# pmh47/dirt

Hardware: AMD Instinct MI355X
Metric: forward+backward Mpixels/s at 1024x1024x4ch, 10k-tri mesh (higher is better)
Workload: dtype f32 (f64 edge functions); 1 GPU; K3: rand_mesh F=10000 at 1024x1024x4, 1 scene(s) per GPU, forward+backward; scenes_per_gpu=1, parallelism=batch-sharded x1, no collective, launch=eager (Python wrapper + C ABI per step)

## Files before the change

### dirt_amd/csrc/dirt_device.h

```cpp
#pragma once
#include <hip/hip_runtime.h>
#include <stdint.h>

namespace dirt {

struct alignas(128) FaceRec {
    double coef[9];
    double inv_det;
    uint32_t flags;
    int32_t vid[3];
    double zp[3];
    uint32_t pad0;
    uint32_t pad1;
};
static_assert(sizeof(FaceRec) == 128, "FaceRec must be 128 bytes");
constexpr int FACE_SHADE_BYTES = 96;

constexpr uint32_t FACE_VALID = 0x80000000u;

struct alignas(8) FaceBox {
    int16_t i_min, i_max, r_min, r_max;
};
static_assert(sizeof(FaceBox) == 8, "FaceBox must be 8 bytes");

constexpr uint32_t Z24_CLEAR = 0x00FFFFFFu;

__device__ __forceinline__ void face_fetch_indices(const int32_t* __restrict__ face, int32_t (&idx)[3])
{
    idx[0] = face[0]; idx[1] = face[1]; idx[2] = face[2];
}
__device__ __forceinline__ void face_fetch_vertices(const float* __restrict__ verts, int V, const int32_t (&idx)[3], float4 (&vv)[3])
{
#pragma unroll
    for (int k = 0; k < 3; ++k)
        vv[k] = V > 0 ? *reinterpret_cast<const float4*>(verts + (size_t)((uint32_t)idx[k] < (uint32_t)V ? idx[k] : 0) * 4) : make_float4(0.f, 0.f, 0.f, 0.f);
}
__device__ inline bool setup_face_from(const float4 (&vv)[3], const int32_t (&idx)[3], int V, int H, int W, FaceRec& rec, FaceBox& box);

__device__ inline bool setup_face(const float* __restrict__ verts, int V, const int32_t* __restrict__ face,
                                  int H, int W, FaceRec& rec, FaceBox& box)
{
    int32_t idx[3];
    float4 vv[3];
    face_fetch_indices(face, idx);
    face_fetch_vertices(verts, V, idx, vv);
    return setup_face_from(vv, idx, V, H, W, rec, box);
}

__device__ inline bool setup_face_edges(const float4 (&vv)[3], const int32_t (&idx)[3], int V, int H, int W, FaceRec& rec)
{
    double X[3], Y[3], Wc[3], Z[3];
    const int32_t i0 = idx[0], i1 = idx[1], i2 = idx[2];
    const bool index_ok = ((uint32_t)i0 < (uint32_t)V) & ((uint32_t)i1 < (uint32_t)V) & ((uint32_t)i2 < (uint32_t)V);
    if (V <= 0) return false;
    if (!index_ok) return false;
#pragma unroll
    for (int k = 0; k < 3; ++k) {
        const int32_t vi = k == 0 ? i0 : (k == 1 ? i1 : i2);
        const float4 v = vv[k];
        if (!(isfinite(v.x) && isfinite(v.y) && isfinite(v.z) && isfinite(v.w))) return false;
        X[k] = ((double)v.x + (double)v.w) * (0.5 * (double)W);
        Y[k] = ((double)v.y + (double)v.w) * (0.5 * (double)H);
        Wc[k] = (double)v.w;
        Z[k] = (double)v.z;
        rec.vid[k] = vi;
    }
    double a[3], b[3], c[3];
#pragma unroll
    for (int k = 0; k < 3; ++k) {
        const int p = (k + 1) % 3, q = (k + 2) % 3;
        double m1, m2;
        m1 = Y[p] * Wc[q]; m2 = Wc[p] * Y[q]; a[k] = m1 - m2;
        m1 = Wc[p] * X[q]; m2 = X[p] * Wc[q]; b[k] = m1 - m2;
        m1 = X[p] * Y[q];  m2 = Y[p] * X[q];  c[k] = m1 - m2;
    }
    const double t0 = X[0] * a[0], t1 = Y[0] * b[0], t2 = Wc[0] * c[0];
    double det = (t0 + t1) + t2;
    if (!isfinite(det) || det == 0.0) return false;
    if (det < 0.0) {
#pragma unroll
        for (int k = 0; k < 3; ++k) { a[k] = -a[k]; b[k] = -b[k]; c[k] = -c[k]; }
        det = -det;
    }
    const double inv_det = 1.0 / det;
    if (!isfinite(inv_det)) return false;

    double zs[3];
#pragma unroll
    for (int k = 0; k < 3; ++k) zs[k] = Z[k] * inv_det;
    {
        double m0, m1, m2;
        m0 = a[0] * zs[0]; m1 = a[1] * zs[1]; m2 = a[2] * zs[2]; rec.zp[0] = ((m0 + m1) + m2) * 8388607.5;
        m0 = b[0] * zs[0]; m1 = b[1] * zs[1]; m2 = b[2] * zs[2]; rec.zp[1] = ((m0 + m1) + m2) * 8388607.5;
        m0 = c[0] * zs[0]; m1 = c[1] * zs[1]; m2 = c[2] * zs[2]; rec.zp[2] = fma((m0 + m1) + m2, 8388607.5, 8388607.5);
    }
    uint32_t flags = FACE_VALID;
#pragma unroll
    for (int k = 0; k < 3; ++k) {
        const bool incl = (a[k] > 0.0) || (a[k] == 0.0 && b[k] > 0.0);
        if (!incl) { a[k] = -a[k]; b[k] = -b[k]; c[k] = -c[k]; flags |= (1u << k); }
        rec.coef[3 * k + 0] = a[k]; rec.coef[3 * k + 1] = b[k]; rec.coef[3 * k + 2] = c[k];
    }
    rec.flags = flags; rec.pad0 = 0; rec.pad1 = 0;
    rec.inv_det = inv_det;
    return true;
}

__device__ inline bool setup_face_box(const float4 (&vv)[3], int H, int W, FaceBox& box)
{
    double X[3], Y[3], Wc[3], Z[3];
#pragma unroll
    for (int k = 0; k < 3; ++k) {
        const float4 v = vv[k];
        X[k] = ((double)v.x + (double)v.w) * (0.5 * (double)W);
        Y[k] = ((double)v.y + (double)v.w) * (0.5 * (double)H);
        Wc[k] = (double)v.w;
        Z[k] = (double)v.z;
    }
    const int npos = (Wc[0] > 0.0) + (Wc[1] > 0.0) + (Wc[2] > 0.0);
    if (npos == 0) return false;
    int i_min = 0, i_max = W - 1, j_min = 0, j_max = H - 1;
    if (npos == 3) {
        if (Z[0] > Wc[0] && Z[1] > Wc[1] && Z[2] > Wc[2]) return false;
        if (Z[0] < -Wc[0] && Z[1] < -Wc[1] && Z[2] < -Wc[2]) return false;
        float xmin = INFINITY, xmax = -INFINITY, ymin = INFINITY, ymax = -INFINITY;
#pragma unroll
        for (int k = 0; k < 3; ++k) {
            const float rw = 1.0f / (float)Wc[k];
            float xw = (float)X[k] * rw, yw = (float)Y[k] * rw;
            if (!(fabsf(xw) <= 32768.f)) xw = xw > 0.f ? 32768.f : -32768.f;
            if (!(fabsf(yw) <= 32768.f)) yw = yw > 0.f ? 32768.f : -32768.f;
            xmin = fminf(xmin, xw); xmax = fmaxf(xmax, xw);
            ymin = fminf(ymin, yw); ymax = fmaxf(ymax, yw);
        }
        if (!(xmin <= xmax) || !(ymin <= ymax)) { xmin = ymin = -32768.f; xmax = ymax = 32768.f; }
        const float d = 1.0f / 32.0f;
        float lo, hi;
        lo = ceilf(fmaxf(xmin - 0.5f - d, -1.0f)); hi = floorf(fminf(xmax - 0.5f + d, (float)W));
        if (lo > (float)i_min) i_min = (int)lo;
        if (hi < (float)i_max) i_max = (int)hi;
        lo = ceilf(fmaxf(ymin - 0.5f - d, -1.0f)); hi = floorf(fminf(ymax - 0.5f + d, (float)H));
        if (lo > (float)j_min) j_min = (int)lo;
        if (hi < (float)j_max) j_max = (int)hi;
    }
    if (i_min > i_max || j_min > j_max) return false;
    box.i_min = (int16_t)i_min; box.i_max = (int16_t)i_max;
    box.r_min = (int16_t)(H - 1 - j_max); box.r_max = (int16_t)(H - 1 - j_min);
    return true;
}

__device__ inline bool setup_face_from(const float4 (&vv)[3], const int32_t (&idx)[3], int V, int H, int W, FaceRec& rec, FaceBox& box)
{
    if (!setup_face_edges(vv, idx, V, H, W, rec)) return false;
    return setup_face_box(vv, H, W, box);
}

__device__ inline void edge_eval(const double* coef, double px, double py, double F[3])
{
    F[0] = fma(coef[0], px, fma(coef[1], py, coef[2]));
    F[1] = fma(coef[3], px, fma(coef[4], py, coef[5]));
    F[2] = fma(coef[6], px, fma(coef[7], py, coef[8]));
}

__device__ inline void bary_eval(const double F[3], uint32_t flags, double inv_det, float b[3], float& clip_w)
{
    const double s0 = (flags & 1u) ? -inv_det : inv_det;
    const double s1 = (flags & 2u) ? -inv_det : inv_det;
    const double s2 = (flags & 4u) ? -inv_det : inv_det;
    const float l0 = (float)(F[0] * s0), l1 = (float)(F[1] * s1), l2 = (float)(F[2] * s2);
    const float s = (l0 + l1) + l2;
    const float r = 1.0f / s;
    b[0] = l0 * r; b[1] = l1 * r; b[2] = l2 * r;
    clip_w = r;
}

__device__ __forceinline__ float2 encode_bary(float b0, float b1, float b2)
{
    const bool omit2 = (b2 >= b0) & (b2 >= b1);
    const bool omit0 = !omit2 & (b0 >= b1);
    const bool omit1 = !omit2 & !omit0;
    const float p = omit2 ? b0 : (omit0 ? b1 : b2);
    const float q = omit2 ? b1 : (omit0 ? b2 : b0);
    return make_float2(__uint_as_float(__float_as_uint(p) | (omit0 ? 0x80000000u : 0u)),
                       __uint_as_float(__float_as_uint(q) | (omit1 ? 0x80000000u : 0u)));
}
__device__ __forceinline__ void decode_bary(float2 e, float (&b)[3])
{
    const bool sp = (int32_t)__float_as_uint(e.x) < 0, sq = (int32_t)__float_as_uint(e.y) < 0;
    const float P = fabsf(e.x), Q = fabsf(e.y);
    const float d = (1.f - P) - Q;
    b[0] = sq ? Q : (sp ? d : P);
    b[1] = sq ? d : (sp ? P : Q);
    b[2] = sq ? P : (sp ? Q : d);
}

__device__ __forceinline__ int xcd_tile(int b, int ntiles)
{
    const int x = b & 7, j = b >> 3;
    const int q = ntiles >> 3, rem = ntiles & 7;
    return x * q + min(x, rem) + j;
}

inline uint32_t tile_magic(int tiles_x) { return tiles_x <= 1 ? 0u : (uint32_t)(0x100000000ull / (uint32_t)tiles_x) + 1u; }
__device__ __forceinline__ void tile_xy(int tile, int tiles_x, uint32_t magic, int& tx, int& ty)
{
    ty = magic ? (int)__umulhi((uint32_t)tile, magic) : tile;
    tx = tile - ty * tiles_x;
}

}
```

### dirt_amd/csrc/dirt_forward.hip

```cpp
#include "dirt_device.h"
#include "dirt_launch.h"
#include "dirt_raster_common.h"
#include "../../include/dirt_hip.h"

namespace dirt {

#ifdef DIRT_TRACE
__device__ long long* g_trace_fwd_setup = nullptr;
__device__ long long* g_trace_fwd_raster = nullptr;
extern "C" void dirt_debug_set_trace_forward(void* ps, void* pr)
{
    long long* q = reinterpret_cast<long long*>(ps);
    (void)hipMemcpyToSymbol(HIP_SYMBOL(g_trace_fwd_setup), &q, sizeof(q));
    q = reinterpret_cast<long long*>(pr);
    (void)hipMemcpyToSymbol(HIP_SYMBOL(g_trace_fwd_raster), &q, sizeof(q));
}
#define FMARK() do { if (tr_n < 12) { long long t_; asm volatile("s_memtime %0\n\ts_waitcnt lgkmcnt(0)" : "=s"(t_) :: "memory"); tr_t[tr_n++] = t_; } } while (0)
#define FTRACE_DECL() long long tr_t[12]; int tr_n = 0; const long long tr_wall0 = wall_clock64()
#else
#define FMARK() do {} while (0)
#define FTRACE_DECL() do {} while (0)
#endif

namespace {

constexpr int MAX_FACE_BINS = 16;

__device__ __forceinline__ void glds16(const void* base, uint32_t voff, uint32_t lds_addr)
{
    unsigned keep;
    asm volatile("s_mov_b32 %0, m0\n\ts_mov_b32 m0, %3\n\ts_nop 0\n\tglobal_load_lds_dwordx4 %1, %2\n\ts_mov_b32 m0, %0"
                 : "=&s"(keep) : "v"(voff), "s"(base), "s"(lds_addr) : "memory");
}

struct Float3v { float x, y, z; };

template <class T>
__device__ __forceinline__ uint32_t lds_address(T* p)
{
    return (uint32_t)(uintptr_t)(__attribute__((address_space(3))) void*)p;
}

}

constexpr int STHREADS = 256;
template <int CK>
__global__ __launch_bounds__(STHREADS) void setup_kernel_v2(const float* __restrict__ a_vertices, const int32_t* __restrict__ a_faces,
                                                            const float* __restrict__ a_vertex_colors, int a_shared_faces, int a_V, int a_F,
                                                            GeomParams g_in)
{
    GeomParams g = g_in;
    g.vertices = a_vertices; g.faces = a_faces; g.vertex_colors = a_vertex_colors; g.shared_faces = a_shared_faces; g.V = a_V; g.F = a_F;
    __shared__ __align__(16) unsigned long long s_mask[MAX_BINS_MASKED + 2];
    __shared__ __align__(16) FaceRec s_recs[64];
    __shared__ __align__(16) TileRec s_lrecs[64];
    __shared__ __align__(16) float4 s_crecs[CK ? 3 * 64 : 1];
    __shared__ FaceBox s_box[64];
    __shared__ uint8_t s_ok_edges[64], s_ok_box[64];
    const int ib = blockIdx.y, chunk = blockIdx.x, tid = threadIdx.x, lane = tid & 63;
    const int role = __builtin_amdgcn_readfirstlane(tid >> 6);
    FTRACE_DECL();
    FMARK();
    const int nbins = g.grid.bins_x * g.grid.bins_y, big = g.grid.big;
    BinCell* __restrict__ row = g.cells + ((size_t)ib * g.nchunk + chunk) * (size_t)g.grid.cell_chunk_stride;
    if (g.F == 0 || g.V <= 0) {
        for (int i = tid; i <= big; i += STHREADS) if (i < nbins || i == big) row[i] = BinCell{0u, 0u};
        return;
    }
    const int f0 = chunk * 64;
    const int nf = min(64, g.F - f0);
    const size_t n0 = (size_t)ib * g.F + f0;
    const int f = f0 + lane;
    const bool have = lane < nf;
    const int fs = have ? f : 0;
    const float* __restrict__ verts = g.vertices + (size_t)ib * g.V * 4;
    const float* __restrict__ cols = CK ? g.vertex_colors + (size_t)ib * g.V * CK : nullptr;
    auto fetch = [&](int vid) {
        if (role != 3) return *reinterpret_cast<const float4*>(verts + (size_t)vid * 4);
        if constexpr (CK == 0) return make_float4(0.f, 0.f, 0.f, 0.f);
        else {
            const float* __restrict__ cp = cols + (size_t)vid * CK;
            if constexpr (CK == 4) return *reinterpret_cast<const float4*>(cp);
            else if constexpr (CK == 3) { const Float3v q = *reinterpret_cast<const Float3v*>(cp); return make_float4(q.x, q.y, q.z, 0.f); }
            else return make_float4(cp[0], 0.f, 0.f, 0.f);
        }
    };
    int32_t idx[3] = {0, 0, 0};
    float4 vv[3];
    const bool fetches = role != 2 && (role != 3 || CK != 0);
    if (fetches) {
        const int32_t* __restrict__ fp = g.faces + (g.shared_faces ? (size_t)fs : (size_t)ib * g.F + fs) * 3;
        idx[0] = fp[0]; idx[1] = fp[1]; idx[2] = fp[2];
#pragma unroll
        for (int k = 0; k < 3; ++k) vv[k] = fetch(min(3 * fs + k, g.V - 1));
    } else if (role == 2) {
        for (int i = lane; i < nbins; i += 64) s_mask[i] = 0ull;
        if (lane == 0) s_mask[big] = 0ull;
    }
    FMARK();
    if (fetches) {
        const bool identity = 3 * fs + 2 < g.V && idx[0] == 3 * fs && idx[1] == 3 * fs + 1 && idx[2] == 3 * fs + 2;
        if (__builtin_amdgcn_ballot_w64(have && !identity) != 0ull) {
#pragma unroll
            for (int k = 0; k < 3; ++k) {
                const int ci = identity ? 3 * fs + k : ((uint32_t)idx[k] < (uint32_t)g.V ? idx[k] : 0);
                vv[k] = fetch(ci);
            }
        }
    }
    FMARK();
    bool ok_mine = false;
    FaceBox box;
    box.i_min = 0; box.i_max = -1; box.r_min = 0; box.r_max = -1;
    if (role == 0) {
        FaceRec rec;
        ok_mine = have && setup_face_edges(vv, idx, g.V, g.H, g.W, rec);
        if (ok_mine) s_recs[lane] = rec;
        else s_recs[lane].flags = 0;
        s_ok_edges[lane] = ok_mine ? 1 : 0;
    } else if (role == 1) {
        ok_mine = have && setup_face_box(vv, g.H, g.W, box);
        s_box[lane] = box;
        s_ok_box[lane] = ok_mine ? 1 : 0;
    } else if (role == 3) {
        if constexpr (CK != 0) { s_crecs[3 * lane] = vv[0]; s_crecs[3 * lane + 1] = vv[1]; s_crecs[3 * lane + 2] = vv[2]; }
    }
    FMARK();
    __syncthreads();
    if (role == 1) {
        if (ok_mine && s_ok_edges[lane]) {
            const unsigned long long bit = 1ull << lane;
            const int bx0 = box.i_min >> g.grid.shift, bx1 = box.i_max >> g.grid.shift;
            const int by0 = box.r_min >> g.grid.shift, by1 = box.r_max >> g.grid.shift;
            if ((bx1 - bx0 + 1) * (by1 - by0 + 1) <= MAX_FACE_BINS) {
                for (int by = by0; by <= by1; ++by)
                    for (int bx = bx0; bx <= bx1; ++bx) atomicOr(&s_mask[by * g.grid.bins_x + bx], bit);
            } else {
                atomicOr(&s_mask[big], bit);
            }
            if (!g.v2_only) {
                BinEntry e;
                e.box = box; e.face = f; e.pad = 0;
                g.entries[((size_t)ib * g.nchunk + chunk) * (5 * (size_t)g.chunk_faces) + lane] = e;
            }
        }
    } else if (role == 2) {
        if (have && s_ok_edges[lane] && s_ok_box[lane]) {
            TileRec lr;
            make_local_rec(s_recs[lane], f, s_box[lane], g.H, (float)g.W, (float)g.H, &lr);
            s_lrecs[lane] = lr;
        }
    } else if (role == 0) {
        const uint4* __restrict__ src = reinterpret_cast<const uint4*>(&s_recs[0]);
        uint4* __restrict__ dst = reinterpret_cast<uint4*>(g.recs + n0);
        for (int i = lane; i < 8 * nf; i += 64) dst[i] = src[i];
    } else {
        if constexpr (CK != 0) {
            const uint4* __restrict__ src = reinterpret_cast<const uint4*>(&s_crecs[0]);
            uint4* __restrict__ dst = reinterpret_cast<uint4*>(g.crecs + 3 * n0);
            for (int i = lane; i < 3 * nf; i += 64) dst[i] = src[i];
        }
    }
    __syncthreads();
    FMARK();
    {
        const uint4* __restrict__ src = reinterpret_cast<const uint4*>(&s_lrecs[0]);
        uint4* __restrict__ dst = reinterpret_cast<uint4*>(g.lrecs + n0);
        for (int i = tid; i < 5 * nf; i += STHREADS) dst[i] = src[i];
    }
    for (int i = 2 * tid; i < nbins; i += 2 * STHREADS) {
        if (i + 1 < nbins) {
            const ulonglong2 m = *reinterpret_cast<const ulonglong2*>(&s_mask[i]);
            *reinterpret_cast<ulonglong2*>(&row[i]) = m;
        } else {
            const unsigned long long m = s_mask[i];
            row[i] = BinCell{(uint32_t)m, (uint32_t)(m >> 32)};
        }
    }
    if (tid == STHREADS - 1) {
        const unsigned long long m = s_mask[big];
        row[big] = BinCell{(uint32_t)m, (uint32_t)(m >> 32)};
    }
    FMARK();
#ifdef DIRT_TRACE
    if (tid == 0 && g_trace_fwd_setup) {
        long long* o = g_trace_fwd_setup + ((size_t)blockIdx.y * gridDim.x + blockIdx.x) * 16;
        for (int i = 0; i < 12; ++i) o[i] = i < tr_n ? tr_t[i] : 0;
        o[12] = tr_wall0; o[13] = (long long)wall_clock64() - tr_wall0;
    }
#endif
}

hipError_t launch_geometry_v2(const GeomParams& g, hipStream_t stream)
{
    const dim3 grid((unsigned)g.nchunk, (unsigned)g.B);
    const int ck = g.crecs ? g.C : 0;
    if (ck == 4) hipLaunchKernelGGL(setup_kernel_v2<4>, grid, dim3(STHREADS), 0, stream, g.vertices, g.faces, g.vertex_colors, g.shared_faces, g.V, g.F, g);
    else if (ck == 3) hipLaunchKernelGGL(setup_kernel_v2<3>, grid, dim3(STHREADS), 0, stream, g.vertices, g.faces, g.vertex_colors, g.shared_faces, g.V, g.F, g);
    else if (ck == 1) hipLaunchKernelGGL(setup_kernel_v2<1>, grid, dim3(STHREADS), 0, stream, g.vertices, g.faces, g.vertex_colors, g.shared_faces, g.V, g.F, g);
    else hipLaunchKernelGGL(setup_kernel_v2<0>, grid, dim3(STHREADS), 0, stream, g.vertices, g.faces, g.vertex_colors, g.shared_faces, g.V, g.F, g);
    return hipGetLastError();
}

namespace {

#ifndef DIRT_V2_CAP
#define DIRT_V2_CAP 96
#endif
constexpr int V2_CAP = DIRT_V2_CAP;

template <bool COLOURS>
struct alignas(16) ShadeSlot {
    double coef[9];
    double inv_det;
    uint32_t flags;
    int32_t vid[3];
    float4 col[COLOURS ? 3 : 0];
};
static_assert(sizeof(ShadeSlot<true>) == 144 && sizeof(ShadeSlot<false>) == 96, "16-byte pieces: 6 of the record, 3 colours");

}

#ifndef DIRT_V2_WAVES
#define DIRT_V2_WAVES 6
#endif
template <int MODE, int CSPEC, int WAVES = 4>
__global__ __launch_bounds__(64 * WAVES, WAVES == 8 ? 8 : DIRT_V2_WAVES) void raster_kernel_v2(
    const BinCell* __restrict__ a_cells, int a_nchunk, int a_tiles_x, int a_tiles_y, uint32_t a_tiles_x_magic, int a_shift, int a_bins_x,
    int a_big, int a_chunk_stride, RasterParams p_in)
{
    RasterParams p = p_in;
    p.cells = a_cells; p.nchunk = a_nchunk; p.tiles_x = a_tiles_x; p.tiles_y = a_tiles_y; p.tiles_x_magic = a_tiles_x_magic;
    p.grid.shift = a_shift; p.grid.bins_x = a_bins_x; p.grid.big = a_big; p.grid.cell_chunk_stride = a_chunk_stride;
    constexpr int NB = 2, NBY = WAVES == 8 ? 1 : 2, TILE = 32, PPL = NB * NBY, THREADS = 64 * WAVES, RH = 8 * NBY;
    constexpr bool COLOURS = MODE == 0;
    constexpr int SPARTS = COLOURS ? 9 : 6;
    using Slot = ShadeSlot<COLOURS>;
    __shared__ __align__(16) TileRec s_rec[V2_CAP];
    __shared__ __align__(16) Slot s_shade[V2_CAP];
    __shared__ int32_t s_face[V2_CAP];
    __shared__ uint32_t s_count;
    FTRACE_DECL();
    FMARK();
#ifdef DIRT_TRACE
    int tr_cand = 0;
#endif
    const int tid = threadIdx.x;
    const int lane = tid & 63;
    const int wave = __builtin_amdgcn_readfirstlane(tid >> 6);
    const int ib = blockIdx.y;
    const int tile = xcd_tile(blockIdx.x, p.tiles_x * p.tiles_y);
    int tile_col, tile_row;
    tile_xy(tile, p.tiles_x, p.tiles_x_magic, tile_col, tile_row);
    const int tx0 = tile_col * TILE, tr0 = tile_row * TILE;
    constexpr int C = CSPEC;

    const FaceRec* __restrict__ recs = p.recs + (size_t)ib * p.F;
    const TileRec* __restrict__ lrecs = p.lrecs + (size_t)ib * p.F;
    const float4* __restrict__ crecs = COLOURS ? p.crecs + (size_t)ib * p.F * 3 : nullptr;
    const int bin = (tr0 >> p.grid.shift) * p.grid.bins_x + (tx0 >> p.grid.shift);
    const BinCell* __restrict__ cells = p.cells + (size_t)ib * p.nchunk * (size_t)p.grid.cell_chunk_stride;
    unsigned long long m_bin = 0ull, m_big = 0ull;
    if (tid < p.nchunk) {
        const BinCell* __restrict__ rowc = cells + (size_t)tid * p.grid.cell_chunk_stride;
        const BinCell a = rowc[bin], b = rowc[p.grid.big];
        m_bin = ((unsigned long long)a.count << 32) | a.start;
        m_big = ((unsigned long long)b.count << 32) | b.start;
    }

    const int wx = wave & 1, wy = wave >> 1;
    const int x0 = tx0 + wx * 16 + (lane & 7);
    const int r0 = tr0 + wy * RH + (lane >> 3);
    double px[NB], py[NBY];
#pragma unroll
    for (int k = 0; k < NB; ++k) px[k] = (double)(x0 + 8 * k) + 0.5;
#pragma unroll
    for (int k = 0; k < NBY; ++k) py[k] = (double)(p.H - 1 - (r0 + 8 * k)) + 0.5;
    unsigned long long best[PPL];
    int cbest[PPL];
#pragma unroll
    for (int k = 0; k < PPL; ++k) { best[k] = (unsigned long long)Z24_CLEAR << 32; cbest[k] = V2_CAP; }
    bool lds_records = true;

    if ((p.zero_b_bytes | p.zero_c_bytes) != 0) {
        const unsigned gwg = blockIdx.y * gridDim.x + blockIdx.x;
        if (p.zero_b_bytes) zero_share<THREADS>(p.zero_b, p.zero_b_bytes, p.zero_b_per, gwg, tid);
        if (p.zero_c_bytes) zero_share<THREADS>(p.zero_c, p.zero_c_bytes, p.zero_c_per, gwg, tid);
    }
    const uint32_t lds_rec = (uint32_t)__builtin_amdgcn_readfirstlane((int)lds_address(&s_rec[0]));
    const uint32_t lds_shade = (uint32_t)__builtin_amdgcn_readfirstlane((int)lds_address(&s_shade[0]));

    FMARK();
    for (int round = 0;; ++round) {
        if (tid == 0) s_count = 0;
        __syncthreads();
        FMARK();
        {
            const uint32_t cnt = (uint32_t)__popcll(m_bin) + (uint32_t)__popcll(m_big);
            uint32_t incl = cnt;
            incl += (uint32_t)__builtin_amdgcn_update_dpp(0, (int)incl, 0x111 , 0xF, 0xF, false);
            incl += (uint32_t)__builtin_amdgcn_update_dpp(0, (int)incl, 0x112 , 0xF, 0xF, false);
            incl += (uint32_t)__builtin_amdgcn_update_dpp(0, (int)incl, 0x114 , 0xF, 0xF, false);
            incl += (uint32_t)__builtin_amdgcn_update_dpp(0, (int)incl, 0x118 , 0xF, 0xF, false);
            incl += (uint32_t)__builtin_amdgcn_update_dpp(0, (int)incl, 0x142 , 0xA, 0xF, false);
            incl += (uint32_t)__builtin_amdgcn_update_dpp(0, (int)incl, 0x143 , 0xC, 0xF, false);
            const uint32_t total = (uint32_t)__builtin_amdgcn_readlane((int)incl, 63);
            uint32_t base = 0;
            if (total != 0u) {
                if (lane == 0) base = atomicAdd(&s_count, total);
                base = (uint32_t)__builtin_amdgcn_readfirstlane((int)base);
            }
            uint32_t slot = base + incl - cnt;
            const int face0 = tid * 64;
            while (m_bin != 0ull && slot < (uint32_t)V2_CAP) {
                s_face[slot++] = face0 + (__ffsll((long long)m_bin) - 1);
                m_bin &= m_bin - 1ull;
            }
            while (m_big != 0ull && slot < (uint32_t)V2_CAP) {
                s_face[slot++] = face0 + (__ffsll((long long)m_big) - 1);
                m_big &= m_big - 1ull;
            }
        }
        FMARK();
        __syncthreads();
        FMARK();
        const int n = (int)min(s_count, (uint32_t)V2_CAP);
        if (round != 0) lds_records = false;

        int tid_o = tid;
        asm volatile("" : "+v"(tid_o));
#pragma unroll
        for (int k = 0; k < (5 * V2_CAP + THREADS - 1) / THREADS; ++k) {
            const int idx = tid_o + THREADS * k;
            if (idx < 5 * n) {
                const int slot = idx / 5, part = idx - 5 * slot;
                glds16(lrecs, (uint32_t)s_face[slot] * (uint32_t)sizeof(TileRec) + 16u * (uint32_t)part, lds_rec + 1024u * (uint32_t)(wave + WAVES * k));
            }
        }
        asm volatile("s_waitcnt vmcnt(0)" ::: "memory");
        FMARK();
        __syncthreads();
        FMARK();
        if (round == 0) {
#pragma unroll
            for (int k = 0; k < (SPARTS * V2_CAP + THREADS - 1) / THREADS; ++k) {
                const int idx = tid_o + THREADS * k;
                if (idx < SPARTS * n) {
                    const int slot = idx / SPARTS, part = idx - SPARTS * slot;
                    const uint32_t face = (uint32_t)s_face[slot];
                    const uint32_t dst = lds_shade + 1024u * (uint32_t)(wave + WAVES * k);
                    if (part < 6) glds16(recs, face * (uint32_t)sizeof(FaceRec) + 16u * (uint32_t)part, dst);
                    if (COLOURS && part >= 6) glds16(crecs, face * 48u + 16u * (uint32_t)(part - 6), dst);
                }
            }
        }

        for (int cb = 0; cb < n; cb += 64) {
            const int idx = cb + lane;
            uint32_t mym4 = 0;
            if (idx < n) {
                const FaceBox box = s_rec[idx].box;
                const int rx0 = tx0 + 16 * wx, ry0 = tr0 + RH * wy;
                const int bx0 = max(box.i_min - rx0, 0) >> 3, bx1 = min(box.i_max - rx0, 15) >> 3;
                const int by0 = max(box.r_min - ry0, 0) >> 3, by1 = min(box.r_max - ry0, RH - 1) >> 3;
                if (box.i_max >= rx0 && box.i_min <= rx0 + 15 && box.r_max >= ry0 && box.r_min <= ry0 + RH - 1) {
                    const uint32_t rowbits = (bx0 == 0 ? 1u : 0u) | (bx1 == 1 ? 2u : 0u);
                    mym4 = (by0 == 0 ? rowbits : 0u) | (NBY == 2 && by1 == 1 ? rowbits << 2 : 0u);
                    mym4 = cull_blocks<NB, NBY>(s_rec[idx], mym4, (float)(rx0 - (int)box.i_min), (float)((int)box.r_min - ry0));
                }
            }
            unsigned long long m = __builtin_amdgcn_ballot_w64(mym4 != 0);
            auto visit = [&](const TileRec& t, int k) {
                const uint32_t m4 = (uint32_t)__builtin_amdgcn_readlane((int)mym4, k);
                float dxl[NB], dyl[NBY];
#pragma unroll
                for (int q = 0; q < NB; ++q) dxl[q] = (float)(x0 + 8 * q - (int)t.box.i_min);
#pragma unroll
                for (int q = 0; q < NBY; ++q) dyl[q] = (float)((int)t.box.r_min - (r0 + 8 * q));
                raster_candidate<NB, NBY>(t, recs, round == 0 ? cb + k : V2_CAP, m4, dxl, dyl, px, py, best, cbest);
#ifdef DIRT_TRACE
                ++tr_cand;
#endif
            };
            while (m) {
                const int k = __ffsll((long long)m) - 1;
                m &= m - 1;
                const TileRec t = s_rec[cb + k];
                visit(t, k);
            }
        }
        FMARK();
        asm volatile("s_waitcnt vmcnt(0)" ::: "memory");
        const bool more = (m_bin | m_big) != 0ull;
        if (!__syncthreads_or(more)) break;
    }
    FMARK();

    int32_t fbest[PPL];
#pragma unroll
    for (int k = 0; k < PPL; ++k) fbest[k] = (uint32_t)(best[k] >> 32) != Z24_CLEAR ? (int32_t)(uint32_t)best[k] : -1;

    constexpr bool BG_FIRST = WAVES != 8;
    const float* __restrict__ cols = COLOURS ? p.vertex_colors + (size_t)ib * p.V * C : nullptr;
    int xs0 = x0, rs0 = r0;
    asm volatile("" : "+v"(xs0), "+v"(rs0));
    auto pixel_index = [&](int k, bool& inside) {
        const int x = xs0 + 8 * (k % NB), r = rs0 + 8 * (k / NB);
        inside = x < p.W && r < p.H;
        return ((size_t)ib * p.H + min(r, p.H - 1)) * p.W + min(x, p.W - 1);
    };
    auto background_at = [&](size_t pix) {
        const float* __restrict__ bg = p.background + pix * C;
        if (CSPEC == 4) return *reinterpret_cast<const float4*>(bg);
        else if (CSPEC == 3) return make_float4(bg[0], bg[1], bg[2], 0.f);
        else return make_float4(bg[0], 0.f, 0.f, 0.f);
    };
    float4 bgv[BG_FIRST ? PPL : 1];
    if constexpr (BG_FIRST) {
#pragma unroll
        for (int k = 0; k < PPL; ++k) {
            bool inside;
            const size_t pix = pixel_index(k, inside);
            bgv[k] = make_float4(0.f, 0.f, 0.f, 0.f);
            if (MODE == 0 && inside && fbest[k] < 0) bgv[k] = background_at(pix);
        }
    }
#pragma unroll
    for (int k = 0; k < PPL; ++k) {
        const int32_t f = fbest[k];
        const bool has = f >= 0;
        const bool from_lds = has && lds_records && cbest[k] < V2_CAP;
        const int ci = from_lds ? cbest[k] : 0;
        double cf[9];
#pragma unroll
        for (int i = 0; i < 9; ++i) cf[i] = s_shade[ci].coef[i];
        uint32_t flags = s_shade[ci].flags;
        double inv_det = s_shade[ci].inv_det;
        const bool from_mem = has && !from_lds;
        const bool any_from_mem = __builtin_amdgcn_ballot_w64(from_mem) != 0ull;
        if (any_from_mem && from_mem) {
            const FaceRec* __restrict__ rec = recs + f;
#pragma unroll
            for (int i = 0; i < 9; ++i) cf[i] = rec->coef[i];
            flags = rec->flags; inv_det = rec->inv_det;
        }
        double Fk[3];
        edge_eval(cf, (double)(xs0 + 8 * (k % NB)) + 0.5, (double)(p.H - 1 - (rs0 + 8 * (k / NB))) + 0.5, Fk);
        float b[3], cw;
        bary_eval(Fk, flags, inv_det, b, cw);
        const float b0 = b[0], b1 = b[1], b2 = b[2];
        bool inside;
        const size_t pix = pixel_index(k, inside);
        if (!inside) continue;
        if (p.vis) p.vis[pix] = f;
        if (p.state_a) store_state(p, pix, has, b0, b1, b2, cw, f);
        if (MODE != 0) continue;
        float4 u0 = make_float4(0.f, 0.f, 0.f, 0.f), u1 = u0, u2 = u0;
        if constexpr (COLOURS) { u0 = s_shade[ci].col[0]; u1 = s_shade[ci].col[1]; u2 = s_shade[ci].col[2]; }
        if (any_from_mem && from_mem) {
            if constexpr (COLOURS) {
                const FaceRec* __restrict__ rec = recs + f;
                const float* __restrict__ c0 = cols + (size_t)rec->vid[0] * C;
                const float* __restrict__ c1 = cols + (size_t)rec->vid[1] * C;
                const float* __restrict__ c2 = cols + (size_t)rec->vid[2] * C;
                if (CSPEC == 4) { u0 = *reinterpret_cast<const float4*>(c0); u1 = *reinterpret_cast<const float4*>(c1); u2 = *reinterpret_cast<const float4*>(c2); }
                else if (CSPEC == 3) { u0 = make_float4(c0[0], c0[1], c0[2], 0.f); u1 = make_float4(c1[0], c1[1], c1[2], 0.f); u2 = make_float4(c2[0], c2[1], c2[2], 0.f); }
                else { u0 = make_float4(c0[0], 0.f, 0.f, 0.f); u1 = make_float4(c1[0], 0.f, 0.f, 0.f); u2 = make_float4(c2[0], 0.f, 0.f, 0.f); }
            }
        }
        float* __restrict__ out = p.pixels + pix * C;
        float4 o;
        if constexpr (BG_FIRST) o = bgv[k];
        else o = has ? make_float4(0.f, 0.f, 0.f, 0.f) : background_at(pix);
        if (has) {
            o.x = fmaf(b2, u2.x, fmaf(b1, u1.x, b0 * u0.x));
            if (CSPEC >= 3) { o.y = fmaf(b2, u2.y, fmaf(b1, u1.y, b0 * u0.y)); o.z = fmaf(b2, u2.z, fmaf(b1, u1.z, b0 * u0.z)); }
            if (CSPEC == 4) o.w = fmaf(b2, u2.w, fmaf(b1, u1.w, b0 * u0.w));
        }
        if (CSPEC == 4) *reinterpret_cast<float4*>(out) = o;
        else if (CSPEC == 3) { out[0] = o.x; out[1] = o.y; out[2] = o.z; }
        else out[0] = o.x;
    }
    FMARK();
#ifdef DIRT_TRACE
    if (lane == 0 && g_trace_fwd_raster) {
        long long* o = g_trace_fwd_raster + (((size_t)blockIdx.y * gridDim.x + blockIdx.x) * WAVES + wave) * 16;
        for (int i = 0; i < 12; ++i) o[i] = i < tr_n ? tr_t[i] : 0;
        o[12] = tr_wall0; o[13] = (long long)wall_clock64() - tr_wall0; o[14] = blockIdx.x; o[15] = tr_cand;
    }
#endif
}

int raster_tile_choice(int H, int W, int B, unsigned flags)
{
    const long long tiles32 = (long long)((W + 31) / 32) * ((H + 31) / 32) * B;
    int tile = tiles32 >= 512 ? 32 : 16;
    if (flags & DIRT_FLAG_TILES_SMALL) tile = 16;
    if (flags & DIRT_FLAG_TILES_LARGE) tile = 32;
    return tile;
}

bool raster_v2_applies(const RasterParams& p, int B, bool visibility_only)
{
    if (!p.masked || p.lrecs == nullptr) return false;
    if (raster_tile_choice(p.H, p.W, B, p.flags) != 32) return false;
    if (visibility_only) return true;
    return (p.C == 1 || p.C == 3 || p.C == 4) && p.crecs != nullptr;
}

hipError_t launch_raster_v2(const RasterParams& p_in, int B, bool visibility_only, hipStream_t stream)
{
    RasterParams p = p_in;
    p.tiles_x = (p.W + 31) / 32;
    p.tiles_y = (p.H + 31) / 32;
    p.tiles_x_magic = tile_magic(p.tiles_x);
    const dim3 grid((unsigned)(p.tiles_x * p.tiles_y), (unsigned)B);
    {
        const size_t nwg = (size_t)grid.x * grid.y;
        p.zero_b_per = (unsigned)((p.zero_b_bytes / 16 + nwg - 1) / nwg);
        p.zero_c_per = (unsigned)((p.zero_c_bytes / 16 + nwg - 1) / nwg);
    }
    const bool pinned8 = (p.flags & (DIRT_FLAG_TILES_LARGE | DIRT_FLAG_TILES_SMALL)) == (DIRT_FLAG_TILES_LARGE | DIRT_FLAG_TILES_SMALL);
    const bool w8 = !visibility_only && (pinned8 || ((size_t)grid.x * grid.y <= 2048 && !(p.flags & DIRT_FLAG_TILES_LARGE)));
#define V2_ARGS p.cells, p.nchunk, p.tiles_x, p.tiles_y, p.tiles_x_magic, p.grid.shift, p.grid.bins_x, p.grid.big, p.grid.cell_chunk_stride, p
    if (visibility_only) hipLaunchKernelGGL((raster_kernel_v2<1, 4>), grid, dim3(RTHREADS), 0, stream, V2_ARGS);
    else if (w8 && p.C == 4) hipLaunchKernelGGL((raster_kernel_v2<0, 4, 8>), grid, dim3(512), 0, stream, V2_ARGS);
    else if (w8 && p.C == 3) hipLaunchKernelGGL((raster_kernel_v2<0, 3, 8>), grid, dim3(512), 0, stream, V2_ARGS);
    else if (w8) hipLaunchKernelGGL((raster_kernel_v2<0, 1, 8>), grid, dim3(512), 0, stream, V2_ARGS);
    else if (p.C == 4) hipLaunchKernelGGL((raster_kernel_v2<0, 4>), grid, dim3(RTHREADS), 0, stream, V2_ARGS);
    else if (p.C == 3) hipLaunchKernelGGL((raster_kernel_v2<0, 3>), grid, dim3(RTHREADS), 0, stream, V2_ARGS);
    else hipLaunchKernelGGL((raster_kernel_v2<0, 1>), grid, dim3(RTHREADS), 0, stream, V2_ARGS);
#undef V2_ARGS
    return hipGetLastError();
}

}
```

### dirt_amd/csrc/dirt_raster_common.h

```cpp
#pragma once
#include "dirt_device.h"
#include "dirt_launch.h"

namespace dirt {

constexpr int RTHREADS = 256;
constexpr int LIST_CAP = 1024;
constexpr int SHADE_CAP = 96;
struct alignas(8) ShadeRec {
    double coef[9];
    double inv_det;
    uint32_t flags;
    int32_t vid[3];
    double pad;
};
static_assert(sizeof(ShadeRec) == 104, "ShadeRec is 26 dwords");

struct alignas(16) TileRec {
    float a[3], b[3], c[3];
    float bound;
    FaceBox box;
    double zp[3];
    uint32_t flags;
    int32_t face;
};
static_assert(sizeof(TileRec) == 80, "TileRec is 80 bytes");

__device__ __forceinline__ void make_tile_rec(const FaceRec& rec, int face, double ox, double oy, float wf, float hf, TileRec* out)
{
    const uint32_t flags = rec.flags;
    float bound = 0.f;
#pragma unroll
    for (int k = 0; k < 3; ++k) {
        const double a = rec.coef[3 * k], b = rec.coef[3 * k + 1], c = rec.coef[3 * k + 2];
        const double cl = fma(a, ox, fma(b, oy, c));
        const float sg = (flags & (1u << k)) ? -1.f : 1.f;
        const float a32 = (float)a, b32 = (float)b, c32 = (float)cl, cg = (float)c;
        const float mg = fabsf(a32) * wf + fabsf(b32) * hf + fabsf(cg);
        const float bnd = (0x1p-22f * (32.f * fabsf(a32) + 32.f * fabsf(b32) + fabsf(c32)) + 0x1p-49f * mg) * 1.0001f;
        bound = (bnd > bound || bnd != bnd) ? bnd : bound;
        out->a[k] = sg * a32; out->b[k] = sg * b32; out->c[k] = sg * c32;
    }
    out->bound = bound; out->box.i_min = 0; out->box.i_max = 0; out->box.r_min = 0; out->box.r_max = 0;
    out->zp[0] = rec.zp[0]; out->zp[1] = rec.zp[1]; out->zp[2] = rec.zp[2];
    out->flags = flags; out->face = face;
}

__device__ __forceinline__ void make_local_rec(const FaceRec& rec, int face, const FaceBox& box, int H, float wf, float hf, TileRec* out)
{
    const uint32_t flags = rec.flags;
    const double ox = (double)box.i_min + 0.5, oy = (double)(H - 1 - box.r_min) + 0.5;
    const float D = (float)(max(box.i_max - box.i_min, box.r_max - box.r_min) + 8);
    float bound = 0.f;
#pragma unroll
    for (int k = 0; k < 3; ++k) {
        const double a = rec.coef[3 * k], b = rec.coef[3 * k + 1], c = rec.coef[3 * k + 2];
        const double cl = fma(a, ox, fma(b, oy, c));
        const float sg = (flags & (1u << k)) ? -1.f : 1.f;
        const float a32 = (float)a, b32 = (float)b, c32 = (float)cl, cg = (float)c;
        const float mg = fabsf(a32) * wf + fabsf(b32) * hf + fabsf(cg);
        const float bnd = (0x1p-22f * (D * fabsf(a32) + D * fabsf(b32) + fabsf(c32)) + 0x1p-49f * mg) * 1.0001f;
        bound = (bnd > bound || bnd != bnd) ? bnd : bound;
        out->a[k] = sg * a32; out->b[k] = sg * b32; out->c[k] = sg * c32;
    }
    out->bound = bound; out->box = box;
    out->zp[0] = rec.zp[0]; out->zp[1] = rec.zp[1]; out->zp[2] = rec.zp[2];
    out->flags = flags; out->face = face;
}

template <int NB, int NBY = NB>
__device__ __forceinline__ uint32_t cull_blocks(const TileRec& t, uint32_t m4, float dx_lo0, float dy_hi0)
{
    const float nb = -t.bound;
#pragma unroll
    for (int by = 0; by < NBY; ++by) {
        const float dy_hi = dy_hi0 - 8.f * (float)by, dy_lo = dy_hi - 7.f;
#pragma unroll
        for (int bx = 0; bx < NB; ++bx) {
            const float dx_lo = dx_lo0 + 8.f * (float)bx, dx_hi = dx_lo + 7.f;
            bool out = false;
#pragma unroll
            for (int k = 0; k < 3; ++k) {
                const float e = fmaf(t.a[k], t.a[k] > 0.f ? dx_hi : dx_lo, fmaf(t.b[k], t.b[k] > 0.f ? dy_hi : dy_lo, t.c[k]));
                out |= e < nb;
            }
            if (out) m4 &= ~(1u << (NB * by + bx));
        }
    }
    return m4;
}

static __device__ __noinline__ bool covered_exact(const FaceRec* __restrict__ rec, double px, double py)
{
    const uint32_t flags = rec->flags;
    const double F0 = fma(rec->coef[0], px, fma(rec->coef[1], py, rec->coef[2]));
    const double F1 = fma(rec->coef[3], px, fma(rec->coef[4], py, rec->coef[5]));
    const double F2 = fma(rec->coef[6], px, fma(rec->coef[7], py, rec->coef[8]));
    return ((F0 >= 0.0) != ((flags & 1u) != 0)) && ((F1 >= 0.0) != ((flags & 2u) != 0)) && ((F2 >= 0.0) != ((flags & 4u) != 0));
}

template <int NB, int NBY = NB>
__device__ __forceinline__ void raster_candidate(const TileRec& t, const FaceRec* __restrict__ recs, int ci, uint32_t m4, const float* dx,
                                                 const float* dy, const double* px, const double* py, unsigned long long* best,
                                                 int* cbest)
{
#pragma unroll
    for (int by = 0; by < NBY; ++by) {
        if (!((m4 >> (NB * by)) & ((1u << NB) - 1u))) continue;
        float trow[3];
        trow[0] = fmaf(t.b[0], dy[by], t.c[0]);
        trow[1] = fmaf(t.b[1], dy[by], t.c[1]);
        trow[2] = fmaf(t.b[2], dy[by], t.c[2]);
        const double qrow = fma(t.zp[1], py[by], t.zp[2]);
#pragma unroll
        for (int bx = 0; bx < NB; ++bx) {
            const int k = NB * by + bx;
            if (!((m4 >> k) & 1u)) continue;
            const float E0 = fmaf(t.a[0], dx[bx], trow[0]);
            const float E1 = fmaf(t.a[1], dx[bx], trow[1]);
            const float E2 = fmaf(t.a[2], dx[bx], trow[2]);
            const float m = fminf(fminf(E0, E1), E2);
            unsigned long long cov_m = __builtin_amdgcn_ballot_w64(m > t.bound);
            const unsigned long long unsure_m = __builtin_amdgcn_ballot_w64(!(m < -t.bound)) & ~cov_m;
            if (__builtin_expect(unsure_m != 0ull, 0)) {
                bool c = false;
                if (__builtin_amdgcn_inverse_ballot_w64(unsure_m)) c = covered_exact(recs + t.face, px[bx], py[by]);
                cov_m |= __builtin_amdgcn_ballot_w64(c);
            }
            if (cov_m == 0ull) continue;
            const double q = fma(t.zp[0], px[bx], qrow);
            const uint32_t z24 = (uint32_t)__double_as_longlong(q + 4503599627370496.0);
            const unsigned long long in_range_m = __builtin_amdgcn_ballot_w64((unsigned long long)__double_as_longlong(q) <= 0x416FFFFFE0000000ull);
            const unsigned long long key = ((unsigned long long)z24 << 32) | (unsigned long long)(uint32_t)t.face;
            const unsigned long long wins_m = cov_m & in_range_m & __builtin_amdgcn_ballot_w64(key < best[k]);
            const bool wins = __builtin_amdgcn_inverse_ballot_w64(wins_m);
            best[k] = wins ? key : best[k];
            cbest[k] = wins ? ci : cbest[k];
        }
    }
}

__device__ __forceinline__ void raster_candidate_pair(const TileRec& t0, const TileRec& t1, const FaceRec* __restrict__ recs, int ci0, int ci1,
                                                      float dx, float dy, double px, double py, unsigned long long& best, int& cbest)
{
    const float E00 = fmaf(t0.a[0], dx, fmaf(t0.b[0], dy, t0.c[0])), E10 = fmaf(t1.a[0], dx, fmaf(t1.b[0], dy, t1.c[0]));
    const float E01 = fmaf(t0.a[1], dx, fmaf(t0.b[1], dy, t0.c[1])), E11 = fmaf(t1.a[1], dx, fmaf(t1.b[1], dy, t1.c[1]));
    const float E02 = fmaf(t0.a[2], dx, fmaf(t0.b[2], dy, t0.c[2])), E12 = fmaf(t1.a[2], dx, fmaf(t1.b[2], dy, t1.c[2]));
    const float m0 = fminf(fminf(E00, E01), E02), m1 = fminf(fminf(E10, E11), E12);
    unsigned long long cov0 = __builtin_amdgcn_ballot_w64(m0 > t0.bound), cov1 = __builtin_amdgcn_ballot_w64(m1 > t1.bound);
    const unsigned long long uns0 = __builtin_amdgcn_ballot_w64(!(m0 < -t0.bound)) & ~cov0, uns1 = __builtin_amdgcn_ballot_w64(!(m1 < -t1.bound)) & ~cov1;
    if (__builtin_expect((uns0 | uns1) != 0ull, 0)) {
        bool c0 = false, c1 = false;
        if (__builtin_amdgcn_inverse_ballot_w64(uns0)) c0 = covered_exact(recs + t0.face, px, py);
        if (__builtin_amdgcn_inverse_ballot_w64(uns1)) c1 = covered_exact(recs + t1.face, px, py);
        cov0 |= __builtin_amdgcn_ballot_w64(c0); cov1 |= __builtin_amdgcn_ballot_w64(c1);
    }
    if ((cov0 | cov1) == 0ull) return;
    const double q0 = fma(t0.zp[0], px, fma(t0.zp[1], py, t0.zp[2])), q1 = fma(t1.zp[0], px, fma(t1.zp[1], py, t1.zp[2]));
    const uint32_t z0 = (uint32_t)__double_as_longlong(q0 + 4503599627370496.0), z1 = (uint32_t)__double_as_longlong(q1 + 4503599627370496.0);
    const unsigned long long in0 = __builtin_amdgcn_ballot_w64((unsigned long long)__double_as_longlong(q0) <= 0x416FFFFFE0000000ull);
    const unsigned long long in1 = __builtin_amdgcn_ballot_w64((unsigned long long)__double_as_longlong(q1) <= 0x416FFFFFE0000000ull);
    const unsigned long long key0 = ((unsigned long long)z0 << 32) | (unsigned long long)(uint32_t)t0.face;
    const unsigned long long key1 = ((unsigned long long)z1 << 32) | (unsigned long long)(uint32_t)t1.face;
    const bool w0 = __builtin_amdgcn_inverse_ballot_w64(cov0 & in0 & __builtin_amdgcn_ballot_w64(key0 < best));
    const unsigned long long b1 = w0 ? key0 : best;
    const int c1i = w0 ? ci0 : cbest;
    const bool w1 = __builtin_amdgcn_inverse_ballot_w64(cov1 & in1 & __builtin_amdgcn_ballot_w64(key1 < b1));
    best = w1 ? key1 : b1;
    cbest = w1 ? ci1 : c1i;
}

__device__ __forceinline__ void store_state(const RasterParams& p, size_t pix, bool has, float b0, float b1, float b2, float clip_w, int32_t face)
{
    p.state_a[pix] = make_float2(has ? clip_w : INFINITY, __int_as_float(face));
    p.state_b[pix] = has ? encode_bary(b0, b1, b2) : make_float2(-1.f, -1.f);
}

template <int NTHREADS = RTHREADS>
__device__ __forceinline__ void zero_share(void* buf, size_t bytes, unsigned per, unsigned gwg, int tid)
{
    const size_t units = bytes / 16;
    const size_t i0 = (size_t)gwg * per;
    uint4* q = reinterpret_cast<uint4*>(buf);
    for (unsigned i = (unsigned)tid; i < per; i += NTHREADS)
        if (i0 + i < units) q[i0 + i] = make_uint4(0u, 0u, 0u, 0u);
    if (gwg == 0 && (size_t)tid < (bytes % 16) / 4) reinterpret_cast<uint32_t*>(buf)[units * 4 + tid] = 0u;
}

}
```

Measured before the change: 23460 Mpixels/s.

## Restructure forward raster shading epilogue and defer scratch zeroing

Reworks the forward raster epilogue in several ways. Background loads are now always issued up front with 32-bit relative offsets from per-tile base pointers. The shading loop is instantiated twice, with and without the global-memory record fallback, chosen by a wave-wide ballot. Colour loads from LDS go through explicit address-space pointers. Zeroing of the gradient scratch buffers moves from kernel start to after shading, and waves with no chunks skip the binning prefix step. bary_eval replaces the double-precision sign selects with float sign-bit XORs. Together these aim to cut address arithmetic, divergent memory branches and early-kernel store traffic, at the cost of extra register pressure from two shade instantiations and the always-prefetched background.

New measurement: 23960 Mpixels/s, median of 6. +2.2%, better.

```diff
diff --git a/dirt_amd/csrc/dirt_device.h b/dirt_amd/csrc/dirt_device.h
--- a/dirt_amd/csrc/dirt_device.h
+++ b/dirt_amd/csrc/dirt_device.h
@@ -164,10 +164,9 @@
 
 __device__ inline void bary_eval(const double F[3], uint32_t flags, double inv_det, float b[3], float& clip_w)
 {
-    const double s0 = (flags & 1u) ? -inv_det : inv_det;
-    const double s1 = (flags & 2u) ? -inv_det : inv_det;
-    const double s2 = (flags & 4u) ? -inv_det : inv_det;
-    const float l0 = (float)(F[0] * s0), l1 = (float)(F[1] * s1), l2 = (float)(F[2] * s2);
+    const float l0 = __uint_as_float(__float_as_uint((float)(F[0] * inv_det)) ^ (flags << 31));
+    const float l1 = __uint_as_float(__float_as_uint((float)(F[1] * inv_det)) ^ ((flags << 30) & 0x80000000u));
+    const float l2 = __uint_as_float(__float_as_uint((float)(F[2] * inv_det)) ^ ((flags << 29) & 0x80000000u));
     const float s = (l0 + l1) + l2;
     const float r = 1.0f / s;
     b[0] = l0 * r; b[1] = l1 * r; b[2] = l2 * r;
diff --git a/dirt_amd/csrc/dirt_forward.hip b/dirt_amd/csrc/dirt_forward.hip
--- a/dirt_amd/csrc/dirt_forward.hip
+++ b/dirt_amd/csrc/dirt_forward.hip
@@ -1,3 +1,4 @@
+#include <type_traits>
 #include "dirt_device.h"
 #include "dirt_launch.h"
 #include "dirt_raster_common.h"
@@ -32,6 +33,21 @@
     asm volatile("s_mov_b32 %0, m0\n\ts_mov_b32 m0, %3\n\ts_nop 0\n\tglobal_load_lds_dwordx4 %1, %2\n\ts_mov_b32 m0, %0"
                  : "=&s"(keep) : "v"(voff), "s"(base), "s"(lds_addr) : "memory");
 }
+
+#define DIRT_LDS __attribute__((address_space(3)))
+
+template <class T>
+__device__ __forceinline__ T ld_at(const void* base, uint32_t off)
+{
+    return *reinterpret_cast<const T*>(reinterpret_cast<const char*>(base) + off);
+}
+template <class T>
+__device__ __forceinline__ void st_at(void* base, uint32_t off, T v)
+{
+    *reinterpret_cast<T*>(reinterpret_cast<char*>(base) + off) = v;
+}
+
+constexpr int WAIT_VMCNT_0 = 0x0F70;
 
 struct Float3v { float x, y, z; };
 
@@ -282,11 +298,6 @@
     for (int k = 0; k < PPL; ++k) { best[k] = (unsigned long long)Z24_CLEAR << 32; cbest[k] = V2_CAP; }
     bool lds_records = true;
 
-    if ((p.zero_b_bytes | p.zero_c_bytes) != 0) {
-        const unsigned gwg = blockIdx.y * gridDim.x + blockIdx.x;
-        if (p.zero_b_bytes) zero_share<THREADS>(p.zero_b, p.zero_b_bytes, p.zero_b_per, gwg, tid);
-        if (p.zero_c_bytes) zero_share<THREADS>(p.zero_c, p.zero_c_bytes, p.zero_c_per, gwg, tid);
-    }
     const uint32_t lds_rec = (uint32_t)__builtin_amdgcn_readfirstlane((int)lds_address(&s_rec[0]));
     const uint32_t lds_shade = (uint32_t)__builtin_amdgcn_readfirstlane((int)lds_address(&s_shade[0]));
 
@@ -295,7 +306,7 @@
         if (tid == 0) s_count = 0;
         __syncthreads();
         FMARK();
-        {
+        if (64 * wave < p.nchunk) {
             const uint32_t cnt = (uint32_t)__popcll(m_bin) + (uint32_t)__popcll(m_big);
             uint32_t incl = cnt;
             incl += (uint32_t)__builtin_amdgcn_update_dpp(0, (int)incl, 0x111 , 0xF, 0xF, false);
@@ -400,86 +411,106 @@
 #pragma unroll
     for (int k = 0; k < PPL; ++k) fbest[k] = (uint32_t)(best[k] >> 32) != Z24_CLEAR ? (int32_t)(uint32_t)best[k] : -1;
 
-    constexpr bool BG_FIRST = WAVES != 8;
     const float* __restrict__ cols = COLOURS ? p.vertex_colors + (size_t)ib * p.V * C : nullptr;
     int xs0 = x0, rs0 = r0;
     asm volatile("" : "+v"(xs0), "+v"(rs0));
-    auto pixel_index = [&](int k, bool& inside) {
+    const size_t row_base = ((size_t)ib * p.H + tr0) * (size_t)p.W;
+    auto pixel_rel = [&](int k, bool& inside) {
         const int x = xs0 + 8 * (k % NB), r = rs0 + 8 * (k / NB);
         inside = x < p.W && r < p.H;
-        return ((size_t)ib * p.H + min(r, p.H - 1)) * p.W + min(x, p.W - 1);
+        return (uint32_t)((min(r, p.H - 1) - tr0) * p.W + min(x, p.W - 1));
     };
-    auto background_at = [&](size_t pix) {
-        const float* __restrict__ bg = p.background + pix * C;
-        if (CSPEC == 4) return *reinterpret_cast<const float4*>(bg);
-        else if (CSPEC == 3) return make_float4(bg[0], bg[1], bg[2], 0.f);
-        else return make_float4(bg[0], 0.f, 0.f, 0.f);
-    };
-    float4 bgv[BG_FIRST ? PPL : 1];
-    if constexpr (BG_FIRST) {
-#pragma unroll
-        for (int k = 0; k < PPL; ++k) {
-            bool inside;
-            const size_t pix = pixel_index(k, inside);
-            bgv[k] = make_float4(0.f, 0.f, 0.f, 0.f);
-            if (MODE == 0 && inside && fbest[k] < 0) bgv[k] = background_at(pix);
-        }
-    }
+    const float* __restrict__ bg_base = MODE == 0 ? p.background + row_base * C : nullptr;
+    float* __restrict__ out_base = MODE == 0 ? p.pixels + row_base * C : nullptr;
+    int32_t* __restrict__ vis_base = p.vis ? p.vis + row_base : nullptr;
+    float2* __restrict__ sa_base = p.state_a ? p.state_a + row_base : nullptr;
+    float2* __restrict__ sb_base = p.state_a ? p.state_b + row_base : nullptr;
+    float4 bgv[PPL];
+#pragma unroll
+    for (int k = 0; k < PPL; ++k) {
+        bool inside;
+        const uint32_t rel = pixel_rel(k, inside);
+        bgv[k] = make_float4(0.f, 0.f, 0.f, 0.f);
+        if (MODE == 0 && inside && fbest[k] < 0) {
+            const uint32_t off = rel * (uint32_t)(C * sizeof(float));
+            if (CSPEC == 4) bgv[k] = ld_at<float4>(bg_base, off);
+            else if (CSPEC == 3) bgv[k] = make_float4(ld_at<float>(bg_base, off), ld_at<float>(bg_base, off + 4u), ld_at<float>(bg_base, off + 8u), 0.f);
+            else bgv[k] = make_float4(ld_at<float>(bg_base, off), 0.f, 0.f, 0.f);
+        }
+    }
+    auto shade = [&](auto mem_tag) {
+    constexpr bool MEM = decltype(mem_tag)::value;
 #pragma unroll
     for (int k = 0; k < PPL; ++k) {
         const int32_t f = fbest[k];
         const bool has = f >= 0;
         const bool from_lds = has && lds_records && cbest[k] < V2_CAP;
         const int ci = from_lds ? cbest[k] : 0;
+        const DIRT_LDS Slot* sl = (const DIRT_LDS Slot*)&s_shade[ci];
         double cf[9];
 #pragma unroll
-        for (int i = 0; i < 9; ++i) cf[i] = s_shade[ci].coef[i];
-        uint32_t flags = s_shade[ci].flags;
-        double inv_det = s_shade[ci].inv_det;
+        for (int i = 0; i < 9; ++i) cf[i] = sl->coef[i];
+        uint32_t flags = sl->flags;
+        double inv_det = sl->inv_det;
         const bool from_mem = has && !from_lds;
-        const bool any_from_mem = __builtin_amdgcn_ballot_w64(from_mem) != 0ull;
-        if (any_from_mem && from_mem) {
-            const FaceRec* __restrict__ rec = recs + f;
-#pragma unroll
-            for (int i = 0; i < 9; ++i) cf[i] = rec->coef[i];
-            flags = rec->flags; inv_det = rec->inv_det;
+        if constexpr (MEM) {
+            if (from_mem) {
+                const FaceRec* __restrict__ rec = recs + f;
+#pragma unroll
+                for (int i = 0; i < 9; ++i) cf[i] = rec->coef[i];
+                flags = rec->flags; inv_det = rec->inv_det;
+            }
         }
         double Fk[3];
         edge_eval(cf, (double)(xs0 + 8 * (k % NB)) + 0.5, (double)(p.H - 1 - (rs0 + 8 * (k / NB))) + 0.5, Fk);
         float b[3], cw;
         bary_eval(Fk, flags, inv_det, b, cw);
         const float b0 = b[0], b1 = b[1], b2 = b[2];
+        float u[3][4] = {};
+        if constexpr (COLOURS) {
+            const DIRT_LDS float* cl = (const DIRT_LDS float*)&s_shade[ci].col[0];
+#pragma unroll
+            for (int i = 0; i < 12; ++i) u[i / 4][i % 4] = cl[i];
+            if constexpr (MEM) {
+                if (from_mem) {
+                    const FaceRec* __restrict__ rec = recs + f;
+#pragma unroll
+                    for (int v = 0; v < 3; ++v) {
+                        const float* __restrict__ cv = cols + (size_t)rec->vid[v] * C;
+#pragma unroll
+                        for (int c = 0; c < C; ++c) u[v][c] = cv[c];
+                    }
+                }
+            }
+        }
+        if (MODE == 0 && k == 0) __builtin_amdgcn_s_waitcnt(WAIT_VMCNT_0);
+        float4 o = bgv[k];
+        if (MODE == 0 && has) {
+            o.x = fmaf(b2, u[2][0], fmaf(b1, u[1][0], b0 * u[0][0]));
+            if (CSPEC >= 3) { o.y = fmaf(b2, u[2][1], fmaf(b1, u[1][1], b0 * u[0][1])); o.z = fmaf(b2, u[2][2], fmaf(b1, u[1][2], b0 * u[0][2])); }
+            if (CSPEC == 4) o.w = fmaf(b2, u[2][3], fmaf(b1, u[1][3], b0 * u[0][3]));
+        }
         bool inside;
-        const size_t pix = pixel_index(k, inside);
+        const uint32_t rel = pixel_rel(k, inside);
         if (!inside) continue;
-        if (p.vis) p.vis[pix] = f;
-        if (p.state_a) store_state(p, pix, has, b0, b1, b2, cw, f);
+        if (p.vis) st_at<int32_t>(vis_base, rel * 4u, f);
+        if (p.state_a) store_state(sa_base, sb_base, rel * 8u, has, b0, b1, b2, cw, f);
         if (MODE != 0) continue;
-        float4 u0 = make_float4(0.f, 0.f, 0.f, 0.f), u1 = u0, u2 = u0;
-        if constexpr (COLOURS) { u0 = s_shade[ci].col[0]; u1 = s_shade[ci].col[1]; u2 = s_shade[ci].col[2]; }
-        if (any_from_mem && from_mem) {
-            if constexpr (COLOURS) {
-                const FaceRec* __restrict__ rec = recs + f;
-                const float* __restrict__ c0 = cols + (size_t)rec->vid[0] * C;
-                const float* __restrict__ c1 = cols + (size_t)rec->vid[1] * C;
-                const float* __restrict__ c2 = cols + (size_t)rec->vid[2] * C;
-                if (CSPEC == 4) { u0 = *reinterpret_cast<const float4*>(c0); u1 = *reinterpret_cast<const float4*>(c1); u2 = *reinterpret_cast<const float4*>(c2); }
-                else if (CSPEC == 3) { u0 = make_float4(c0[0], c0[1], c0[2], 0.f); u1 = make_float4(c1[0], c1[1], c1[2], 0.f); u2 = make_float4(c2[0], c2[1], c2[2], 0.f); }
-                else { u0 = make_float4(c0[0], 0.f, 0.f, 0.f); u1 = make_float4(c1[0], 0.f, 0.f, 0.f); u2 = make_float4(c2[0], 0.f, 0.f, 0.f); }
-            }
-        }
-        float* __restrict__ out = p.pixels + pix * C;
-        float4 o;
-        if constexpr (BG_FIRST) o = bgv[k];
-        else o = has ? make_float4(0.f, 0.f, 0.f, 0.f) : background_at(pix);
-        if (has) {
-            o.x = fmaf(b2, u2.x, fmaf(b1, u1.x, b0 * u0.x));
-            if (CSPEC >= 3) { o.y = fmaf(b2, u2.y, fmaf(b1, u1.y, b0 * u0.y)); o.z = fmaf(b2, u2.z, fmaf(b1, u1.z, b0 * u0.z)); }
-            if (CSPEC == 4) o.w = fmaf(b2, u2.w, fmaf(b1, u1.w, b0 * u0.w));
-        }
-        if (CSPEC == 4) *reinterpret_cast<float4*>(out) = o;
-        else if (CSPEC == 3) { out[0] = o.x; out[1] = o.y; out[2] = o.z; }
-        else out[0] = o.x;
+        const uint32_t off = rel * (uint32_t)(C * sizeof(float));
+        if (CSPEC == 4) st_at<float4>(out_base, off, o);
+        else if (CSPEC == 3) { st_at<float>(out_base, off, o.x); st_at<float>(out_base, off + 4u, o.y); st_at<float>(out_base, off + 8u, o.z); }
+        else st_at<float>(out_base, off, o.x);
+    }
+    };
+    bool some_from_mem = false;
+#pragma unroll
+    for (int k = 0; k < PPL; ++k) some_from_mem |= fbest[k] >= 0 && !(lds_records && cbest[k] < V2_CAP);
+    if (__builtin_amdgcn_ballot_w64(some_from_mem) != 0ull) shade(std::true_type());
+    else shade(std::false_type());
+    if ((p.zero_b_bytes | p.zero_c_bytes) != 0) {
+        const unsigned gwg = blockIdx.y * gridDim.x + blockIdx.x;
+        if (p.zero_b_bytes) zero_share<THREADS>(p.zero_b, p.zero_b_bytes, p.zero_b_per, gwg, tid);
+        if (p.zero_c_bytes) zero_share<THREADS>(p.zero_c, p.zero_c_bytes, p.zero_c_per, gwg, tid);
     }
     FMARK();
 #ifdef DIRT_TRACE
diff --git a/dirt_amd/csrc/dirt_raster_common.h b/dirt_amd/csrc/dirt_raster_common.h
--- a/dirt_amd/csrc/dirt_raster_common.h
+++ b/dirt_amd/csrc/dirt_raster_common.h
@@ -170,10 +170,14 @@
     cbest = w1 ? ci1 : c1i;
 }
 
+__device__ __forceinline__ void store_state(float2* plane_a, float2* plane_b, uint32_t off, bool has, float b0, float b1, float b2, float clip_w, int32_t face)
+{
+    *reinterpret_cast<float2*>(reinterpret_cast<char*>(plane_a) + off) = make_float2(has ? clip_w : INFINITY, __int_as_float(face));
+    *reinterpret_cast<float2*>(reinterpret_cast<char*>(plane_b) + off) = has ? encode_bary(b0, b1, b2) : make_float2(-1.f, -1.f);
+}
 __device__ __forceinline__ void store_state(const RasterParams& p, size_t pix, bool has, float b0, float b1, float b2, float clip_w, int32_t face)
 {
-    p.state_a[pix] = make_float2(has ? clip_w : INFINITY, __int_as_float(face));
-    p.state_b[pix] = has ? encode_bary(b0, b1, b2) : make_float2(-1.f, -1.f);
+    store_state(p.state_a + pix, p.state_b + pix, 0u, has, b0, b1, b2, clip_w, face);
 }
 
 template <int NTHREADS = RTHREADS>
```
